# Tung-I/Dual-awareness-Attention-for-Few-shot-Object-Detection

Hardware: AMD Instinct MI355X
Metric: query-images/sec (res50, way=2, shot=3, bs=4 per GPU, train-mode forward) (higher is better)
Workload: dtype f32 (operands, accumulation, results; multiplies as an exact bf16x3 split, six bf16 MFMA products each)

## Files before the change

dual-awareness-attention-for-few-shot-object-detection_amd/csrc/attention.hip:

```cpp
#include "common.h"
#include "../../include/dana_hip.h"
#include "attn_segments.h"
#include <float.h>

namespace {

__device__ __forceinline__ float wave_sum(float v) {
#pragma unroll
  for (int o = 32; o > 0; o >>= 1) v += __shfl_xor(v, o);
  return v;
}
__device__ __forceinline__ float wave_max(float v) {
#pragma unroll
  for (int o = 32; o > 0; o >>= 1) v = fmaxf(v, __shfl_xor(v, o));
  return v;
}

__global__ void __launch_bounds__(256)
rowdot_kernel(const float* __restrict__ x, const float* __restrict__ w, const float* __restrict__ bias,
              float* __restrict__ out, long rows, int D, long ld) {
  const int lane = threadIdx.x & 63;
  const long row = (long)blockIdx.x * 4 + (threadIdx.x >> 6);
  if (row >= rows) return;
  const float4* xr = (const float4*)(x + row * ld);
// ... 25 lines not shown
  }
  s = wave_sum(s);
  for (int l = lane; l < L; l += 64) r[l] = r[l] / s;
}

__global__ void __launch_bounds__(256)
ba_apply_kernel(float* __restrict__ S, const float* __restrict__ w, int L, int D, long ld, float gamma, float slope) {
  extern __shared__ float ws[];
  float* part = ws + ((L + 3) & ~3);
  const int g = blockIdx.y;
  for (int l = threadIdx.x; l < L; l += blockDim.x) ws[l] = w[(long)g * L + l];
  __syncthreads();
  const int c4 = threadIdx.x & 15, rg = threadIdx.x >> 4;
  const int d = blockIdx.x * 64 + c4 * 4;
  const bool ok = d + 3 < D;
  float* base = S + (long)g * L * ld + d;
  float4 acc = make_float4(0.f, 0.f, 0.f, 0.f);
  if (ok)
    for (int l = rg; l < L; l += 16) {
      const float4 v = *(const float4*)(base + (long)l * ld);
      const float wl = ws[l];
      acc.x += wl * v.x;
      acc.y += wl * v.y;
      acc.z += wl * v.z;
      acc.w += wl * v.w;
    }
  *(float4*)(part + rg * 64 + c4 * 4) = acc;
  __syncthreads();
  float4 tot = make_float4(0.f, 0.f, 0.f, 0.f);
#pragma unroll
  for (int r = 0; r < 16; ++r) {
    const float4 p = *(const float4*)(part + r * 64 + c4 * 4);
    tot.x += p.x;
    tot.y += p.y;
    tot.z += p.z;
    tot.w += p.w;
  }
  float4 add;
  add.x = gamma * (tot.x > 0.f ? tot.x : tot.x * slope);
  add.y = gamma * (tot.y > 0.f ? tot.y : tot.y * slope);
  add.z = gamma * (tot.z > 0.f ? tot.z : tot.z * slope);
  add.w = gamma * (tot.w > 0.f ? tot.w : tot.w * slope);
  if (ok)
    for (int l = rg; l < L; l += 16) {
      float4 v = *(const float4*)(base + (long)l * ld);
      v.x += add.x;
      v.y += add.y;
      v.z += add.z;
      v.w += add.w;
      *(float4*)(base + (long)l * ld) = v;
    }
}

__global__ void __launch_bounds__(256)
attn_softmax_unary_kernel(float* __restrict__ scores, const float* __restrict__ unary, long rows, long rows_per_batch,
                          long unary_batch_stride, int nseg, int L, long ld, int kpad, float ugamma, float out_scale) {
  const int lane = threadIdx.x & 63;
  const long row = (long)blockIdx.x * 4 + (threadIdx.x >> 6);
  if (row >= rows) return;
  float* r = scores + row * ld;
  const float* u = unary + (row / rows_per_batch) * unary_batch_stride;
  constexpr int RV = 8;
  if (L <= 64 * RV) {
    for (int sgm = 0; sgm < nseg; ++sgm) {
      float* x = r + sgm * L;
      float v[RV];
      float m = -FLT_MAX;
#pragma unroll
      for (int i = 0; i < RV; ++i) {
        const int l = lane + 64 * i;
        v[i] = l < L ? x[l] : -FLT_MAX;
        m = fmaxf(m, v[i]);
      }
      m = wave_max(m);
      float s = 0.f;
#pragma unroll
      for (int i = 0; i < RV; ++i)
        if (lane + 64 * i < L) {
          v[i] = expf(v[i] - m);
          s += v[i];
        }
      s = wave_sum(s);
#pragma unroll
      for (int i = 0; i < RV; ++i) {
        const int l = lane + 64 * i;
        if (l < L) x[l] = (v[i] / s + ugamma * u[sgm * L + l]) * out_scale;
      }
    }
    for (int l = nseg * L + lane; l < kpad; l += 64) r[l] = 0.f;
    return;
  }
  for (int sgm = 0; sgm < nseg; ++sgm) {
    float* x = r + sgm * L;
    float m = -FLT_MAX;
    for (int l = lane; l < L; l += 64) m = fmaxf(m, x[l]);
    m = wave_max(m);
    float s = 0.f;
    for (int l = lane; l < L; l += 64) {
      const float e = expf(x[l] - m);
      x[l] = e;
      s += e;
    }
    s = wave_sum(s);
    for (int l = lane; l < L; l += 64) x[l] = (x[l] / s + ugamma * u[sgm * L + l]) * out_scale;
  }
  for (int l = nseg * L + lane; l < kpad; l += 64) r[l] = 0.f;
// ... 13 lines not shown
}

}

extern "C" {

int dana_rowdot(const float* x, const float* w, const float* bias, float* out, long rows, int dim, long ld,
                dana_stream_t stream) {
  DANA_CHECK_ARG(rows >= 0 && dim > 0 && dim % 4 == 0, "dana_rowdot: bad shape");
  if (rows == 0) return DANA_OK;
  DANA_CHECK_ARG(x && w && out, "dana_rowdot: null pointer");
  if (ld <= 0) ld = dim;
  DANA_CHECK_ARG(ld % 4 == 0, "dana_rowdot: ld %% 4 != 0");
  rowdot_kernel<<<dana_ceil_div(rows, 4), 256, 0, (hipStream_t)stream>>>(x, w, bias, out, rows, dim, ld);
  DANA_CHECK_LAUNCH("dana_rowdot");
  return DANA_OK;
}

int dana_softmax_rows(float* x, long groups, int length, long ld, dana_stream_t stream) {
  DANA_CHECK_ARG(groups >= 0 && length > 0, "dana_softmax_rows: bad shape");
  if (groups == 0) return DANA_OK;
  DANA_CHECK_ARG(x, "dana_softmax_rows: null pointer");
  if (ld <= 0) ld = length;
  softmax_rows_kernel<<<dana_ceil_div(groups, 4), 256, 0, (hipStream_t)stream>>>(x, groups, length, ld);
  DANA_CHECK_LAUNCH("dana_softmax_rows");
  return DANA_OK;
}

int dana_softmax_rows_to(const float* x, float* out, long groups, int length, long ld_in, long ld_out, dana_stream_t stream) {
  DANA_CHECK_ARG(groups >= 0 && length > 0, "dana_softmax_rows_to: bad shape");
  if (groups == 0) return DANA_OK;
  DANA_CHECK_ARG(x && out, "dana_softmax_rows_to: null pointer");
  if (ld_in <= 0) ld_in = length;
  if (ld_out <= 0) ld_out = length;
  softmax_rows_kernel<<<dana_ceil_div(groups, 4), 256, 0, (hipStream_t)stream>>>(out, groups, length, ld_out, x, ld_in);
  DANA_CHECK_LAUNCH("dana_softmax_rows_to");
  return DANA_OK;
}

int dana_ba_apply(float* s, const float* w, int groups, int length, int dim, long ld, float gamma, float slope,
                  dana_stream_t stream) {
  DANA_CHECK_ARG(groups >= 0 && length > 0 && dim > 0, "dana_ba_apply: bad shape");
  if (groups == 0) return DANA_OK;
  DANA_CHECK_ARG(s && w, "dana_ba_apply: null pointer");
  if (ld <= 0) ld = dim;
  DANA_CHECK_ARG(dim % 4 == 0 && ld % 4 == 0 && ((uintptr_t)s & 15) == 0, "dana_ba_apply: dim, ld must be multiples of 4 (float4 rows)");
  dim3 grid(dana_ceil_div(dim, 64), groups);
  const size_t lds = (size_t)(((length + 3) & ~3) + 16 * 64) * sizeof(float);
  ba_apply_kernel<<<grid, 256, lds, (hipStream_t)stream>>>(s, w, length, dim, ld, gamma, slope);
  DANA_CHECK_LAUNCH("dana_ba_apply");
  return DANA_OK;
}

int dana_attn_softmax_unary(float* scores, const float* unary, long rows, long rows_per_batch, long unary_batch_stride,
                            int nseg, int length, long ld, int kpad, float unary_gamma, float out_scale,
                            dana_stream_t stream) {
  DANA_CHECK_ARG(rows >= 0 && rows_per_batch > 0 && nseg > 0 && length > 0 && ld >= (long)nseg * length &&
                     kpad <= ld,
                 "dana_attn_softmax_unary: bad shape");
  if (rows == 0) return DANA_OK;
  DANA_CHECK_ARG(scores && unary, "dana_attn_softmax_unary: null pointer");
  attn_softmax_unary_kernel<<<dana_ceil_div(rows, 4), 256, 0, (hipStream_t)stream>>>(
      scores, unary, rows, rows_per_batch, unary_batch_stride > 0 ? unary_batch_stride : (long)nseg * length, nseg,
      length, ld, kpad, unary_gamma, out_scale);
  DANA_CHECK_LAUNCH("dana_attn_softmax_unary");
  return DANA_OK;
}

int dana_attn_softmax_unary_w(float* scores, const float* unary, long rows, long rows_per_batch, long unary_batch_stride,
                              int nseg, int length, long ld, int kpad, float unary_gamma, const float* seg_scale,
                              long scale_batch_stride, dana_stream_t stream) {
  DANA_CHECK_ARG(rows >= 0 && rows_per_batch > 0 && nseg > 0 && length > 0 && ld >= (long)nseg * length &&
                     kpad <= ld,
                 "dana_attn_softmax_unary_w: bad shape");
  if (rows == 0) return DANA_OK;
  DANA_CHECK_ARG(scores && unary && seg_scale, "dana_attn_softmax_unary_w: null pointer");
  attn_softmax_unary_w_kernel<<<dana_ceil_div(rows, 4), 256, 0, (hipStream_t)stream>>>(
      scores, unary, seg_scale, rows, rows_per_batch, unary_batch_stride > 0 ? unary_batch_stride : (long)nseg * length,
      scale_batch_stride > 0 ? scale_batch_stride : (long)nseg, nseg, length, ld, kpad, unary_gamma);
  DANA_CHECK_LAUNCH("dana_attn_softmax_unary_w");
  return DANA_OK;
}

}
```

dual-awareness-attention-for-few-shot-object-detection_amd/csrc/elementwise.hip:

```cpp
#include "common.h"
#include "../../include/dana_hip.h"
#include <float.h>

namespace {

int grid_for(long total, int block) {
  long g = (total + block - 1) / block;
  return (int)(g < 1 ? 1 : (g > 65535L * 16 ? 65535L * 16 : g));
}

__global__ void __launch_bounds__(256)
nchw_to_nhwc_kernel(const float* __restrict__ in, float* __restrict__ out, int C, int HW, int cpad, long ldo,
                    long total) {
  for (long i = (long)blockIdx.x * blockDim.x + threadIdx.x; i < total; i += (long)blockDim.x * gridDim.x) {
    const int c = (int)(i % cpad);
    const long pix = i / cpad;
    const long b = pix / HW, hw = pix % HW;
    out[pix * ldo + c] = c < C ? in[(b * C + c) * HW + hw] : 0.f;
  }
}

__global__ void __launch_bounds__(256)
nchw3_to_nhwc4_kernel(const float* __restrict__ in, float4* __restrict__ out, int HW, int total_pix) {
  for (int i = blockIdx.x * blockDim.x + threadIdx.x; i < total_pix; i += blockDim.x * gridDim.x) {
// ... 292 lines not shown
    for (int dy = 0; dy < k; ++dy) {
      const float4 v = hsum[((oy + dy) * OW + ox) * AP_CH4 + q];
      s.x += v.x;
      s.y += v.y;
      s.z += v.z;
      s.w += v.w;
    }
    out[((b * OH + oy) * OW + ox) * C4 + c0 + q] = make_float4(s.x * inv, s.y * inv, s.z * inv, s.w * inv);
  }
}

__global__ void __launch_bounds__(256)
spatial_mean_kernel(const float4* __restrict__ in, float4* __restrict__ out, int P, int C4, long ldi4, long total) {
  const float cnt = (float)P;
  for (long i = (long)blockIdx.x * blockDim.x + threadIdx.x; i < total; i += (long)blockDim.x * gridDim.x) {
    const int c = (int)(i % C4);
    const long g = i / C4;
    float4 s = make_float4(0, 0, 0, 0);
    for (int p = 0; p < P; ++p) {
      const float4 v = in[(g * P + p) * ldi4 + c];
      s.x += v.x;
      s.y += v.y;
      s.z += v.z;
      s.w += v.w;
    }
    out[i] = make_float4(s.x / cnt, s.y / cnt, s.z / cnt, s.w / cnt);
  }
}

__global__ void __launch_bounds__(256)
add_pe_kernel(const float4* __restrict__ in, const float4* __restrict__ pe, float4* __restrict__ out, int L, int C4,
              long ldi4, long ldo4, long total) {
  for (long i = (long)blockIdx.x * blockDim.x + threadIdx.x; i < total; i += (long)blockDim.x * gridDim.x) {
    const int c = (int)(i % C4);
    const long r = i / C4;
    const float4 a = in[r * ldi4 + c], b = pe[(r % L) * C4 + c];
    out[r * ldo4 + c] = make_float4(a.x + b.x, a.y + b.y, a.z + b.z, a.w + b.w);
  }
}

__global__ void __launch_bounds__(256)
add_pe_groups_kernel(const float4* __restrict__ in, const float4* __restrict__ pe, float4* __restrict__ out, int L, int C4,
                     long rows_per_group, long in_group4, long out_group4, long total) {
  for (long i = (long)blockIdx.x * blockDim.x + threadIdx.x; i < total; i += (long)blockDim.x * gridDim.x) {
    const int c = (int)(i % C4);
    const long rr = i / C4;
    const long g = rr / rows_per_group, r = rr % rows_per_group;
    const float4 a = in[g * in_group4 + r * C4 + c], b = pe[(r % L) * C4 + c];
    out[g * out_group4 + r * C4 + c] = make_float4(a.x + b.x, a.y + b.y, a.z + b.z, a.w + b.w);
  }
}

constexpr int CM_ROWS = 64;
__global__ void __launch_bounds__(256)
colmean_partial_kernel(const float* __restrict__ x, float* __restrict__ partial, int L, int D, long ld) {
  __shared__ float part[4][64];
  const int col = blockIdx.x * 64 + (threadIdx.x & 63);
  const int rl = threadIdx.x >> 6;
  const float* base = x + (long)blockIdx.z * L * ld;
  const int l0 = blockIdx.y * CM_ROWS, l1 = min(L, l0 + CM_ROWS);
  float s = 0.f;
  if (col < D)
    for (int l = l0 + rl; l < l1; l += 4) s += base[(long)l * ld + col];
  part[rl][threadIdx.x & 63] = s;
  __syncthreads();
  if (rl == 0 && col < D)
    partial[((long)blockIdx.z * gridDim.y + blockIdx.y) * D + col] =
        (part[0][threadIdx.x] + part[1][threadIdx.x]) + (part[2][threadIdx.x] + part[3][threadIdx.x]);
}
__global__ void __launch_bounds__(256)
colmean_apply_kernel(float* __restrict__ x, const float* __restrict__ partial, int L, int D, long ld) {
  const int col = blockIdx.x * 64 + (threadIdx.x & 63);
  const int rl = threadIdx.x >> 6;
  if (col >= D) return;
  float s = 0.f;
  for (int c = 0; c < (int)gridDim.y; ++c) s += partial[((long)blockIdx.z * gridDim.y + c) * D + col];
  const float mean = s / (float)L;
  float* base = x + (long)blockIdx.z * L * ld;
  const int l0 = blockIdx.y * CM_ROWS, l1 = min(L, l0 + CM_ROWS);
  for (int l = l0 + rl; l < l1; l += 4) base[(long)l * ld + col] -= mean;
}

__global__ void __launch_bounds__(256)
colmean_fused_kernel(float* __restrict__ x, int L, int D, long ld) {
  __shared__ float part[4][64];
  __shared__ float mean_s[64];
  const int tc = threadIdx.x & 63, col = blockIdx.x * 64 + tc, rl = threadIdx.x >> 6;
  float* base = x + (long)blockIdx.z * L * ld;
  float total = 0.f;
  for (int l0 = 0; l0 < L; l0 += CM_ROWS) {
    const int l1 = min(L, l0 + CM_ROWS);
    float s = 0.f;
    if (col < D)
      for (int l = l0 + rl; l < l1; l += 4) s += base[(long)l * ld + col];
    part[rl][tc] = s;
    __syncthreads();
    if (rl == 0) total += (part[0][tc] + part[1][tc]) + (part[2][tc] + part[3][tc]);
    __syncthreads();
  }
  if (rl == 0) mean_s[tc] = total / (float)L;
  __syncthreads();
  if (col >= D) return;
  const float mean = mean_s[tc];
  for (int l = rl; l < L; l += 4) base[(long)l * ld + col] -= mean;
}

__global__ void __launch_bounds__(256)
transpose_kernel(const float* __restrict__ in, float* __restrict__ out, int R, int C, long ldi, long ldo,
                 long in_batch, long out_batch, int zero_pad) {
  __shared__ float t[32][33];
  const float* ib = in + (long)blockIdx.z * in_batch;
  float* ob = out + (long)blockIdx.z * out_batch;
  const int c0 = blockIdx.x * 32, r0 = blockIdx.y * 32;
  const int tx = threadIdx.x & 31, ty = threadIdx.x >> 5;
  for (int j = ty; j < 32; j += 8) {
    const int r = r0 + j, c = c0 + tx;
    t[j][tx] = (r < R && c < C) ? ib[(long)r * ldi + c] : 0.f;
  }
  __syncthreads();
  for (int j = ty; j < 32; j += 8) {
    const int c = c0 + j, r = r0 + tx;
    if (c < C && (r < R || (zero_pad && r < ldo))) ob[(long)c * ldo + r] = t[tx][j];
  }
}

__global__ void __launch_bounds__(256)
labels_posneg_kernel(const float* __restrict__ labels, long long* __restrict__ out, long n) {
  const long i = (long)blockIdx.x * blockDim.x + threadIdx.x;
  if (i >= 2 * n) return;
  out[i] = i < n ? (long long)labels[i] : 0ll;
}

__global__ void __launch_bounds__(256)
bn_train_backward_kernel(const float* __restrict__ dy, const float* __restrict__ x, const float* __restrict__ mean,
                         const float* __restrict__ var, const float* __restrict__ gamma, float eps, long rows, int C,
                         float* __restrict__ dx, float* __restrict__ dgamma, float* __restrict__ dbeta, int accumulate) {
  __shared__ float s1[4][64], s2[4][64];
  const int cl = threadIdx.x & 63, rl = threadIdx.x >> 6;
  const int c = blockIdx.x * 64 + cl;
  const bool ok = c < C;
  const float mu = ok ? mean[c] : 0.f;
  const float istd = ok ? 1.0f / sqrtf(var[c] + eps) : 0.f;
  float a1 = 0.f, a2 = 0.f;
  if (ok)
    for (long r = rl; r < rows; r += 4) {
      const float g = dy[r * C + c];
      a1 += g;
      a2 += g * ((x[r * C + c] - mu) * istd);
    }
  s1[rl][cl] = a1;
  s2[rl][cl] = a2;
  __syncthreads();
  const float t1 = ((s1[0][cl] + s1[1][cl]) + s1[2][cl]) + s1[3][cl];
  const float t2 = ((s2[0][cl] + s2[1][cl]) + s2[2][cl]) + s2[3][cl];
  if (!ok) return;
  if (rl == 0) {
    dgamma[c] = accumulate ? dgamma[c] + t2 : t2;
// ... 291 lines not shown
        (const float4*)in, (float4*)out, height, width, oh, ow, channels / 4, k, rows_total);
  } else {
    avgpool_kernel<<<grid_for(total, 256), 256, 0, (hipStream_t)stream>>>((const float4*)in, (float4*)out, height, width,
                                                                          oh, ow, channels / 4, k, stride, total);
  }
  DANA_CHECK_LAUNCH("dana_avgpool_nhwc");
  return DANA_OK;
}

int dana_spatial_mean_nhwc(const float* in, float* out, int groups, int positions, int channels, long in_pix_stride,
                           dana_stream_t stream) {
  DANA_CHECK_ARG(groups >= 0 && positions > 0 && channels % 4 == 0, "dana_spatial_mean_nhwc: bad shape");
  if (groups == 0) return DANA_OK;
  DANA_CHECK_ARG(in && out, "dana_spatial_mean_nhwc: null pointer");
  if (in_pix_stride <= 0) in_pix_stride = channels;
  DANA_CHECK_ARG(in_pix_stride % 4 == 0, "dana_spatial_mean_nhwc: stride %% 4 != 0");
  const long total = (long)groups * (channels / 4);
  spatial_mean_kernel<<<grid_for(total, 256), 256, 0, (hipStream_t)stream>>>(
      (const float4*)in, (float4*)out, positions, channels / 4, in_pix_stride / 4, total);
  DANA_CHECK_LAUNCH("dana_spatial_mean_nhwc");
  return DANA_OK;
}

int dana_add_pe(const float* in, const float* pe, float* out, long rows, int length, int channels,
                long in_stride, long out_stride, dana_stream_t stream) {
  DANA_CHECK_ARG(rows >= 0 && length > 0 && channels > 0 && channels % 4 == 0, "dana_add_pe: bad shape");
  if (rows == 0) return DANA_OK;
  DANA_CHECK_ARG(in && pe && out, "dana_add_pe: null pointer");
  if (in_stride <= 0) in_stride = channels;
  if (out_stride <= 0) out_stride = channels;
  DANA_CHECK_ARG(in_stride % 4 == 0 && out_stride % 4 == 0, "dana_add_pe: strides %% 4 != 0");
  const long total = rows * (channels / 4);
  add_pe_kernel<<<grid_for(total, 256), 256, 0, (hipStream_t)stream>>>(
      (const float4*)in, (const float4*)pe, (float4*)out, length, channels / 4, in_stride / 4, out_stride / 4, total);
  DANA_CHECK_LAUNCH("dana_add_pe");
  return DANA_OK;
}

int dana_add_pe_groups(const float* in, const float* pe, float* out, long groups, long rows_per_group, int length, int channels,
                       long in_group_stride, long out_group_stride, dana_stream_t stream) {
  DANA_CHECK_ARG(groups >= 0 && rows_per_group > 0 && length > 0 && channels > 0 && channels % 4 == 0 &&
                     in_group_stride % 4 == 0 && out_group_stride % 4 == 0,
                 "dana_add_pe_groups: bad shape");
  if (groups == 0) return DANA_OK;
  DANA_CHECK_ARG(in && pe && out, "dana_add_pe_groups: null pointer");
  const long total = groups * rows_per_group * (channels / 4);
  add_pe_groups_kernel<<<grid_for(total, 256), 256, 0, (hipStream_t)stream>>>(
      (const float4*)in, (const float4*)pe, (float4*)out, length, channels / 4, rows_per_group, in_group_stride / 4,
      out_group_stride / 4, total);
  DANA_CHECK_LAUNCH("dana_add_pe_groups");
  return DANA_OK;
}

size_t dana_colmean_sub_workspace_bytes(int groups, int length, int dim) {
  if (groups <= 0 || length <= 0 || dim <= 0) return 0;
  return (size_t)groups * ((length + CM_ROWS - 1) / CM_ROWS) * dim * sizeof(float);
}

int dana_colmean_sub(float* x, int groups, int length, int dim, long ld, void* workspace, size_t workspace_bytes,
                     dana_stream_t stream) {
  DANA_CHECK_ARG(groups >= 0 && length > 0 && dim > 0, "dana_colmean_sub: bad shape");
  if (groups == 0) return DANA_OK;
  DANA_CHECK_ARG(x, "dana_colmean_sub: null pointer");
  if (ld <= 0) ld = dim;
  const size_t need = dana_colmean_sub_workspace_bytes(groups, length, dim);
  if (!workspace || workspace_bytes < need) {
    dana_set_error("dana_colmean_sub: workspace %zu < %zu", workspace_bytes, need);
    return DANA_ERR_WORKSPACE;
  }
  if (length <= 1024 && groups <= 65535) {
    dim3 grid1(dana_ceil_div(dim, 64), 1, groups);
    colmean_fused_kernel<<<grid1, 256, 0, (hipStream_t)stream>>>(x, length, dim, ld);
    DANA_CHECK_LAUNCH("dana_colmean_sub(fused)");
    return DANA_OK;
  }
  dim3 grid(dana_ceil_div(dim, 64), dana_ceil_div(length, CM_ROWS), groups);
  DANA_CHECK_ARG(grid.y <= 65535 && grid.z <= 65535, "dana_colmean_sub: too many chunks/groups");
  colmean_partial_kernel<<<grid, 256, 0, (hipStream_t)stream>>>(x, (float*)workspace, length, dim, ld);
  DANA_CHECK_LAUNCH("dana_colmean_sub(partial)");
  colmean_apply_kernel<<<grid, 256, 0, (hipStream_t)stream>>>(x, (const float*)workspace, length, dim, ld);
  DANA_CHECK_LAUNCH("dana_colmean_sub(apply)");
  return DANA_OK;
}

int dana_transpose_batched(const float* in, float* out, int groups, int rows, int cols, long ldi, long ldo,
                           long in_batch, long out_batch, dana_stream_t stream) {
  DANA_CHECK_ARG(groups >= 0 && rows > 0 && cols > 0 && ldi >= cols && ldo >= rows, "dana_transpose_batched: bad shape");
  if (groups == 0) return DANA_OK;
  DANA_CHECK_ARG(in && out, "dana_transpose_batched: null pointer");
  const int zero_pad = ldo > rows ? 1 : 0;
  dim3 grid(dana_ceil_div(cols, 32), dana_ceil_div(zero_pad ? (int)ldo : rows, 32), groups);
  transpose_kernel<<<grid, 256, 0, (hipStream_t)stream>>>(in, out, rows, cols, ldi, ldo, in_batch, out_batch, zero_pad);
  DANA_CHECK_LAUNCH("dana_transpose_batched");
  return DANA_OK;
}

int dana_labels_posneg_i64(const float* labels, long long* out, long n, dana_stream_t stream) {
  DANA_CHECK_ARG(n >= 0, "dana_labels_posneg_i64: bad shape");
  if (n == 0) return DANA_OK;
  DANA_CHECK_ARG(labels && out, "dana_labels_posneg_i64: null pointer");
  labels_posneg_kernel<<<dana_ceil_div(2 * n, 256), 256, 0, (hipStream_t)stream>>>(labels, out, n);
  DANA_CHECK_LAUNCH("dana_labels_posneg_i64");
  return DANA_OK;
}

int dana_pack_conv_weight(const float* w_oihw, float* out, int cout, int cin, int kh, int kw, int stem7,
                          dana_stream_t stream) {
  DANA_CHECK_ARG(cout > 0 && cin > 0 && kh > 0 && kw > 0, "dana_pack_conv_weight: bad shape");
  DANA_CHECK_ARG(w_oihw && out, "dana_pack_conv_weight: null pointer");
  if (stem7) {
    DANA_CHECK_ARG(kh == 7 && kw == 7 && cin <= 4, "dana_pack_conv_weight: stem7 needs 7x7, cin<=4");
    const long total = (long)cout * 224;
    pack_stem_kernel<<<grid_for(total, 256), 256, 0, (hipStream_t)stream>>>(w_oihw, out, cin, total);
  } else {
    const long total = (long)cout * cin * kh * kw;
    pack_weight_kernel<<<grid_for(total, 256), 256, 0, (hipStream_t)stream>>>(w_oihw, out, cin, kh, kw, total);
  }
  DANA_CHECK_LAUNCH("dana_pack_conv_weight");
  return DANA_OK;
}

// ... 47 lines not shown
```

dual-awareness-attention-for-few-shot-object-detection_amd/dana.py:

```python
import contextlib
import math
import time
import weakref
from types import SimpleNamespace

import numpy as np
import torch
import torch.nn as nn
import torch.nn.functional as F

from . import ops
from .config import cfg
from . import targets as T


class Bottleneck(nn.Module):
    expansion = 4

    def __init__(self, inplanes, planes, stride=1, downsample=None):
        super().__init__()
        self.conv1 = nn.Conv2d(inplanes, planes, kernel_size=1, stride=stride, bias=False)
        self.bn1 = nn.BatchNorm2d(planes)
        self.conv2 = nn.Conv2d(planes, planes, kernel_size=3, stride=1, padding=1, bias=False)
        self.bn2 = nn.BatchNorm2d(planes)
# ... 84 lines not shown
                               "(each forward can be differentiated once; run the forward again)")
        gs = [torch.zeros((), device=fctx.model._grad_anchor.device) if g is None else g.reshape(()) for g in (g1, g2, g3, g4)]
        fctx.saved = None
        BW.model_backward(fctx.model, torch.stack(gs), ctx=ctx)
        return None, None, None, None, None, None


_HERE = contextlib.nullcontext()

ATTENTION_LEVELS = ("ba", "rpn", "roi")


def _on(stream):
    return _HERE if stream is None else ops.on_stream(stream)


def _rows(t, row):
    return t[row:] if row and t is not None else t


class DAnARCNN(nn.Module):

    def __init__(self, classes, attention_type="concat", rpn_reduce_dim=256, rcnn_reduce_dim=256, gamma=0.1,
                 semantic_enhance=False, num_layers=50, pretrained=False, num_way=2, num_shot=5, pos_encoding=True):
        super().__init__()
        if attention_type not in ("concat", "product"):
            raise ValueError("attention_type must be 'concat' or 'product' (dana.py:70-77)")
        self.model_path = "data/pretrained_model/resnet50_caffe.pth"
        self.dout_base_model = 1024
        self.pretrained = pretrained
        self.classes = classes
        self.n_classes = len(classes)
        self.n_way = num_way
        self.n_shot = num_shot
        self.attention_type = attention_type
        self.channel_gamma = gamma
        self.unary_gamma = 0.1
        self.semantic_enhance = semantic_enhance
        self.rpn_reduce_dim = rpn_reduce_dim
        self.rcnn_reduce_dim = rcnn_reduce_dim
        self.pos_encoding = pos_encoding
        self.pool_feat_dim = 1024
        self.rcnn_dim = 64
        self.use_winograd = True
        self.winograd_tile = 4
        self.winograd_min_cin = 128
        self.presplit_weights = True
        self.merge_trunk = False
        self.merge_from = 0
        self.fold_roi_pe = True
        self.fold_roi_attn = True
        self.prefetch_dgrad = "layer4"
        self.rpn_side_role = "wgrad"
        self.nms_inclusive = False
        dim_in = self.pool_feat_dim

        def lin(i, o):
            m = nn.Linear(i, o)
            nn.init.normal_(m.weight, std=0.01)
            nn.init.constant_(m.bias, 0)
            return m

        self.rpn_unary_layer = lin(dim_in, 1)
        self.rcnn_unary_layer = lin(dim_in, 1)
        self.rpn_adapt_q_layer = lin(dim_in, rpn_reduce_dim)
        self.rpn_adapt_k_layer = lin(dim_in, rpn_reduce_dim)
        self.rcnn_adapt_q_layer = lin(dim_in, rcnn_reduce_dim)
        self.rcnn_adapt_k_layer = lin(dim_in, rcnn_reduce_dim)
        if self.semantic_enhance:
            self.rpn_channel_k_layer = lin(dim_in, 1)
        corr_dim = 2048 if attention_type == "concat" else 1024
        self.RCNN_rpn = _RPNParams(corr_dim)
        self.rcnn_transform_layer = nn.Linear(corr_dim, self.rcnn_dim)
        self.output_score_layer = FFN(64 * 49, dim_in)
        self._plan = None
        self._consts = {}
        self.generalised_support = False
        self.device_rng = False
        self.rng_seed = 1996
        self._rng_calls = 0
        self._conv_cache = {}
        self._epoch = 0
        self._ctx = None
        self._grad_anchor = None

    def create_architecture(self):
        self._init_modules()
        self._init_weights()

    trunk_layers = (3, 4, 6, 3)

    def _init_modules(self):
        resnet = _ResNet50Params(tuple(self.trunk_layers))
        if self.pretrained:
            print("Loading pretrained weights from %s" % (self.model_path))
            state_dict = torch.load(self.model_path)
            resnet.load_state_dict({k: v for k, v in state_dict.items() if k in resnet.state_dict()})
        self.RCNN_base = nn.Sequential(resnet.conv1, resnet.bn1, resnet.relu, resnet.maxpool, resnet.layer1,
                                       resnet.layer2, resnet.layer3)
        self.RCNN_top = nn.Sequential(resnet.layer4)
        self.RCNN_bbox_pred = nn.Linear(2048, 4)
        for p in self.RCNN_base[0].parameters():
            p.requires_grad = False
        for p in self.RCNN_base[1].parameters():
            p.requires_grad = False
        assert 0 <= cfg.RESNET.FIXED_BLOCKS < 4
# ... 370 lines not shown
            if side is not None:
                main.wait_event(ops.record_event(side))
            return [(n, hw, row, None) for n, hw, row, _ in segs]

        merged = two and merge_from <= 0
        segs, row = [], 0
        for i, im in enumerate(ims):
            n, _, H, W = im.shape
            segs.append((n, (H, W), row, side if i and not merged else None))
            row += n * H * W
        x, segs = self._stem(segs, ims, plan["stem"], merged, alloc)
        yield
        nl = len(plan["layers"])
        stall = getattr(self, "_debug_stall", None) if two else None
        for li, layer in enumerate(plan["layers"]):
            if two and not merged and li >= merge_from:
                segs, merged = join(segs), True
            for bi, bp in enumerate(layer):
                last = (li == nl - 1) and (bi == len(layer) - 1)
                if stall is not None and not merged and li == stall[0]:
                    torch.cuda._sleep(int(stall[1]))
                x, segs, dest = self._block(segs, x, bp, merged, outs=outs if last and outs[0][1] else None,
                                            saves=saves if li >= save_from else None, key="RCNN_base.%d.%d" % (4 + li, bi), alloc=alloc,
                                            save_m=save_m)
                if not last:
                    yield
        if two and not merged:
            segs = join(segs)
        return x, segs, dest

    @staticmethod
    def _feat_size(H, W):
        h, w = (H + 6 - 7) // 2 + 1, (W + 6 - 7) // 2 + 1
        h, w = ops.maxpool_out_size(h, w)
        for _ in range(2):
            h, w = (h - 1) // 2 + 1, (w - 1) // 2 + 1
        return h, w

    def _check_support_map(self, sh_, sw_):
        if (sh_, sw_) != (20, 20):
            if not self.generalised_support or sh_ % 7 or sw_ % 7:
                raise RuntimeError("support images must be 320x320 (20x20 stride-16 map), as the reference hard-codes "
                                   "(dana.py:105); got a %dx%d map%s" % (sh_, sw_, "" if self.generalised_support else
                                   " (set model.generalised_support = True for maps whose sides are multiples of 7)"))

    def _support_rpn_side(self, sup, B, shot, way, L, dev, stream, ctx=None, branch=True, tap=None):
        s_pe = torch.empty((B, shot * L, 1024), dtype=torch.float32, device=dev)
        ops.add_pe_groups(sup, self._pe_table(L, dev), B, shot * L, L, 1024, way * shot * L * 1024, s_pe)
        return self._support_rpn_chain(s_pe, B, shot, L, dev, stream, ctx, branch, tap)

    def _support_rpn_chain(self, s_pe, B, shot, L, dev, stream, ctx=None, branch=True, tap=None):
        d = self.rpn_reduce_dim
        K1 = shot * L
        if self.semantic_enhance:
            wc, bc = self._w(self.rpn_channel_k_layer)
            wgt = ops.rowdot(s_pe, wc, bc, B * shot * L, 1024)
            ops.softmax_rows_(wgt, B * shot, L)
            if ctx is not None:
                ctx.update(s_pre=s_pe.clone(), ba_w=wgt)
            if tap is not None:
                tap["ba_w"] = wgt
            ops.ba_apply_(s_pe, wgt, B * shot, L, 1024, gamma=self.channel_gamma, slope=0.01)
        br_role = getattr(self, "rpn_side_role", "wgrad")
        br = self._stream(br_role, dev) if (branch and br_role and not getattr(self, "_single_stream", False)
                                            and not torch.cuda.is_current_stream_capturing()) else None

        def unary_and_transpose():
            wu, bu = self._w(self.rpn_unary_layer)
            u_ = ops.rowdot(s_pe, wu, bu, B * shot * L, 1024)
            ops.softmax_rows_(u_, B * shot, L)
            return u_, ops.transpose_batched(s_pe, B, K1, 1024)

        if br is not None:
            s_pe_ready = ops.record_event()
            br.wait_event(s_pe_ready)
            s_pe.record_stream(br)
            with ops.on_stream(br):
                unary, s_t = unary_and_transpose()
                branch_done = ops.record_event()
        _, bk = self._w(self.rpn_adapt_k_layer)
        kb3, kld = self._lin_b(self.rpn_adapt_k_layer)
        kp = ops.gemm_nt(s_pe, kb3, B * shot * L, d, 1024, ldb=kld, shift=bk)
        ops.colmean_sub_(kp, B * shot, L, d)
        if br is not None:
            stream.wait_event(branch_done)
        else:
            unary, s_t = unary_and_transpose()
        return s_pe, kp, unary, s_t

    def _support_roi_side(self, sup, Ns, sh_, sw_, plan, dev, product, ctx=None):
        P2 = cfg.POOLING_SIZE * cfg.POOLING_SIZE
        pool = self._support_pool(sh_, sw_)
        sp = ops.avgpool(sup, Ns, sh_, sw_, 1024, pool[0], pool[1])
        sp_pe = ops.add_pe(sp, plan["pe49"], Ns * P2, P2, 1024)
        k2, un2, sw = self._support_roi_chain(sp_pe, Ns, product, ctx)
        return sp_pe, k2, un2, sw, pool

    @staticmethod
    def _support_pool(sh_, sw_):
        if (sh_, sw_) == (20, 20):
            return (14, 1)
        if sh_ != sw_:
            raise RuntimeError("generalised supports must be square")
        return (sh_ // 7, sh_ // 7)

    def _support_roi_chain(self, sp_pe, Ns, product, ctx=None):
        P2 = cfg.POOLING_SIZE * cfg.POOLING_SIZE
        dq = self.rcnn_reduce_dim
        _, bk2 = self._w(self.rcnn_adapt_k_layer)
        k2b3, k2ld = self._lin_b(self.rcnn_adapt_k_layer)
        k2 = ops.gemm_nt(sp_pe, k2b3, Ns * P2, dq, 1024, ldb=k2ld, shift=bk2)
        ops.colmean_sub_(k2, Ns, P2, dq)
        wu2, bu2 = self._w(self.rcnn_unary_layer)
        un2 = ops.rowdot(sp_pe, wu2, bu2, Ns * P2, 1024)
        ops.softmax_rows_(un2, Ns, P2)
        sw = None
        if getattr(self, "fold_roi_attn", True) and not product:
            wt_a_s, wt_a_s_ld = self._lin_b(self.rcnn_transform_layer, 1024, 1024)
            sw = ops.gemm_nt(sp_pe, wt_a_s, Ns * P2, self.rcnn_dim, 1024, ldb=wt_a_s_ld)
            if ctx is not None:
                ctx["sw"] = sw
        return k2, un2, sw

    def _rpn_split_plan(self, plan):
# ... 1113 lines not shown
```

dual-awareness-attention-for-few-shot-object-detection_amd/ops.py:

```python
import ctypes
import time as _time

import torch

from ._lib import lib, DanaError

HOST_WAIT = [0.0]

NCHW, NHWC = 0, 1
EPI_RELU, CONV_STEM7, W_SPLIT3, A_SPLIT3 = 1, 2, 256, 512

PROFILE = None
PROF_ROLE = None


def _prof_begin():
    if PROFILE is None:
        return None
    e = torch.cuda.Event(enable_timing=True)
    e.record()
    return e


def _prof_end(e0, tag, flops, nbytes=0.0, executed=None):
# ... 1032 lines not shown
        if v is not None and v.data_ptr() == w.data_ptr():
            return _chk(v, "weight")
    w = _chk(w.detach().contiguous(), "weight")
    O, I, KH, KW = w.shape
    out = torch.empty((O, 7 * 8 * 4) if stem else (O, KH * KW * I), dtype=torch.float32, device=w.device)
    lib().call("dana_pack_conv_weight", _p(w), _p(out), O, I, KH, KW, int(stem), _stream())
    return out


def bn_fold(bn_weight, bn_bias, running_mean, running_var, eps):
    n = bn_weight.numel()
    scale = torch.empty((n,), dtype=torch.float32, device=bn_weight.device)
    shift = torch.empty_like(scale)
    lib().call("dana_bn_fold", _p(_chk(bn_weight.detach().contiguous(), "gamma")),
               _p(_chk(bn_bias.detach().contiguous(), "beta")), _p(_chk(running_mean.contiguous(), "mean")),
               _p(_chk(running_var.contiguous(), "var")), float(eps), _p(scale), _p(shift), n, _stream())
    return scale, shift


def rowdot(x, w, bias, rows, dim, ld=0):
    _chk(x, "x")
    out = torch.empty((rows,), dtype=torch.float32, device=x.device)
    lib().call("dana_rowdot", _p(x), _p(_chk(w.detach().contiguous(), "w")),
               _p(_chk(bias.detach().contiguous(), "bias")) if bias is not None else None, _p(out), rows, dim, ld,
               _stream())
    return out


def softmax_rows_(x, groups, length, ld=0):
    _chk(x, "x")
    lib().call("dana_softmax_rows", _p(x), groups, length, ld, _stream())
    return x


def softmax_rows_to(x, out, groups, length, ld_in=0, ld_out=0):
    lib().call("dana_softmax_rows_to", _p(_chk(x, "x")), _p(_chk(out, "out")), groups, length, ld_in, ld_out, _stream())
    return out


def labels_posneg(labels_f):
    n = labels_f.numel()
    out = torch.empty(2 * n, dtype=torch.int64, device=labels_f.device)
    lib().call("dana_labels_posneg_i64", _p(_chk(labels_f, "labels")), _p(out), n, _stream())
    return out


def ba_apply_(s, w, groups, length, dim, ld=0, gamma=0.1, slope=0.01):
    _chk(s, "s")
    _chk(w, "w")
    lib().call("dana_ba_apply", _p(s), _p(w), groups, length, dim, ld, float(gamma), float(slope), _stream())
    return s


def attn_softmax_unary_(scores, unary, rows, rows_per_batch, nseg, length, ld, kpad, unary_gamma, out_scale,
                        unary_batch_stride=0):
    _chk(scores, "scores")
    _chk(unary, "unary")
    lib().call("dana_attn_softmax_unary", _p(scores), _p(unary), rows, rows_per_batch, unary_batch_stride, nseg, length,
               ld, kpad,
               float(unary_gamma), float(out_scale), _stream())
    return scores


def attn_softmax_unary_w_(scores, unary, rows, rows_per_batch, nseg, length, ld, kpad, unary_gamma, seg_scale,
                          unary_batch_stride=0, scale_batch_stride=0):
    _chk(scores, "scores")
    _chk(unary, "unary")
    _chk(seg_scale, "seg_scale")
    lib().call("dana_attn_softmax_unary_w", _p(scores), _p(unary), rows, rows_per_batch, unary_batch_stride, nseg, length,
               ld, kpad, float(unary_gamma), _p(seg_scale), scale_batch_stride, _stream())
    return scores


def attn_softmax_unary_sweep_w(scores, out, unary, B, C, hw, nseg, length, ld_in, ld_out, kpad, unary_gamma, seg_scale,
                               unary_stride=0, scale_stride=0):
    _chk(scores, "scores")
    _chk(out, "out")
    _chk(unary, "unary")
    _chk(seg_scale, "seg_scale")
    lib().call("dana_attn_softmax_unary_sweep_w", _p(scores), _p(out), _p(unary), B, C, hw, unary_stride, nseg, length,
               ld_in, ld_out, kpad, float(unary_gamma), _p(seg_scale), scale_stride, _stream())
    return out


def gather_shot_blocks(srcs, rows, blocks, index, view, m):
    P, shot, dev = index.numel(), view.size(1), index.device
    _chk(index, "index", torch.int32)
    _chk(view, "view", torch.int32)
    for t, r, b in zip(srcs, rows, blocks):
        _chk(t, "src")
        if t.numel() != t.size(0) * r * shot * b:
            raise ValueError("gather_shot_blocks: a source is not [n_sets][%d][%d][%d]" % (r, shot, b))
    dsts = [torch.empty((P, r, m, b), dtype=torch.float32, device=dev) for r, b in zip(rows, blocks)]
    w = torch.empty((P, m), dtype=torch.float32, device=dev)
    tab = torch.tensor([[t.data_ptr() for t in srcs], [t.data_ptr() for t in dsts], list(rows), [b * 4 for b in blocks]],
                       dtype=torch.int64).to(dev)
    lib().call("dana_gather_shot_blocks", _p(tab[0]), _p(tab[1]), _p(tab[2]), _p(tab[3]), len(srcs), _p(index), _p(view),
               _p(w), srcs[0].size(0), shot, m, P, _stream())
    return dsts, w


def bank_gather_episode(map_pe, pool_pe, index, B, way, shot, s_pe=None, sp_pe=None):
    _chk(map_pe, "map_pe")
    _chk(pool_pe, "pool_pe")
    _chk(index, "index", torch.int32)
    if map_pe.dim() != 3 or pool_pe.dim() != 3 or pool_pe.size(0) != map_pe.size(0) or pool_pe.size(2) != map_pe.size(2):
# ... 411 lines not shown
```

include/dana_hip.h:

```cpp
#ifndef DANA_HIP_H
#define DANA_HIP_H
#include <stddef.h>
#include <stdint.h>

#ifdef __cplusplus
extern "C" {
#endif

typedef void* dana_stream_t;

#define DANA_LAYOUT_NCHW 0
#define DANA_LAYOUT_NHWC 1

#define DANA_EPI_RELU 1
#define DANA_CONV_STEM7 2
#define DANA_W_SPLIT3 256
#define DANA_A_SPLIT3 512

const char* dana_last_error(void);
int dana_abi_version(void);

int dana_set_mfma_mode(int mode);
int dana_get_mfma_mode(void);

// ... 171 lines not shown
                                dana_stream_t stream);
int dana_avgpool_nhwc(const float* in, float* out, int batch, int height, int width, int channels, int k, int stride,
                      dana_stream_t stream);
int dana_spatial_mean_nhwc(const float* in, float* out, int groups, int positions, int channels, long in_pix_stride,
                           dana_stream_t stream);
int dana_batch_stats(const float* x, float* mean, float* var_biased, long rows, int channels, long ld, void* workspace,
                     size_t workspace_bytes, dana_stream_t stream);
int dana_scale_shift_relu(float* x, const float* scale, const float* shift, long rows, int channels, int relu,
                          dana_stream_t stream);
int dana_bn_train_backward(const float* grad_out, const float* x, const float* mean, const float* var_biased,
                           const float* gamma, float eps, long rows, int channels, float* grad_x, float* grad_gamma,
                           float* grad_beta, int accumulate, dana_stream_t stream);
int dana_depthwise_corr_nhwc(const float* feat, const float* kernels, float* out, long n_maps, int height, int width,
                             int channels, int kh, int kw, long maps_per_kernel, long feat_pix_stride,
                             dana_stream_t stream);
int dana_depthwise_corr_nhwc_grouped(const float* feat, const float* kernels, float* out, long n_maps, int height,
                                     int width, int channels, int kh, int kw, int group, long feat_pix_stride,
                                     dana_stream_t stream);
int dana_depthwise_corr_backward_nhwc(const float* grad_out, const float* feat, const float* kernels, float* grad_feat,
                                      float* grad_kernels, long n_maps, int height, int width, int channels, int kh,
                                      int kw, long maps_per_kernel, long feat_pix_stride, int accumulate_kernels,
                                      dana_stream_t stream);
int dana_maxpool2x2s2_nhwc(const float* in, float* out, int batch, int height, int width, int channels,
                           dana_stream_t stream);
int dana_maxpool2x2s2_backward_nhwc(const float* in, const float* grad_out, float* grad_in, int batch, int height,
                                    int width, int channels, dana_stream_t stream);
int dana_sigmoid(float* x, long n, dana_stream_t stream);
int dana_scale_rows_by_group(const float* x, const float* group_vec, float* out, long rows, long rows_per_group,
                             int channels, dana_stream_t stream);
int dana_scale_rows_grouped(const float* x, const float* vec, float* out, long rows, int channels, long ld_x, int group,
                            long n_blocks, dana_stream_t stream);
int dana_add_pe(const float* in, const float* pe, float* out, long rows, int length, int channels,
                long in_stride, long out_stride, dana_stream_t stream);
int dana_add_pe_groups(const float* in, const float* pe, float* out, long groups, long rows_per_group, int length, int channels,
                       long in_group_stride, long out_group_stride, dana_stream_t stream);
size_t dana_colmean_sub_workspace_bytes(int groups, int length, int dim);
int dana_colmean_sub(float* x, int groups, int length, int dim, long ld, void* workspace, size_t workspace_bytes,
                     dana_stream_t stream);
int dana_transpose_batched(const float* in, float* out, int groups, int rows, int cols, long ldi, long ldo,
                           long in_batch, long out_batch, dana_stream_t stream);
int dana_pack_conv_weight(const float* w_oihw, float* out, int cout, int cin, int kh, int kw, int stem7,
                          dana_stream_t stream);
int dana_bn_fold(const float* gamma, const float* beta, const float* mean, const float* var, float eps, float* scale,
                 float* shift, int n, dana_stream_t stream);


int dana_rowdot(const float* x, const float* w, const float* bias, float* out, long rows, int dim, long ld,
                dana_stream_t stream);
int dana_softmax_rows(float* x, long groups, int length, long ld, dana_stream_t stream);
int dana_softmax_rows_to(const float* x, float* out, long groups, int length, long ld_in, long ld_out, dana_stream_t stream);
int dana_labels_posneg_i64(const float* labels, long long* out, long n, dana_stream_t stream);
int dana_ba_apply(float* s, const float* w, int groups, int length, int dim, long ld, float gamma, float slope,
                  dana_stream_t stream);
int dana_attn_softmax_unary(float* scores, const float* unary, long rows, long rows_per_batch, long unary_batch_stride,
                            int nseg, int length, long ld, int kpad, float unary_gamma, float out_scale,
                            dana_stream_t stream);
int dana_attn_softmax_unary_w(float* scores, const float* unary, long rows, long rows_per_batch, long unary_batch_stride,
                              int nseg, int length, long ld, int kpad, float unary_gamma, const float* seg_scale,
                              long scale_batch_stride, dana_stream_t stream);


int dana_proposal_target_prepare(const float* rois, const float* gt_boxes, int B, int n_rois, int n_gt,
                                 float fg_thresh, float bg_thresh_hi, float bg_thresh_lo, float* max_overlaps,
                                 int* gt_assignment, int* fg_list, int* bg_list, int* counts, dana_stream_t stream);
int dana_proposal_target_gather(const float* rois, const float* gt_boxes, int B, int n_rois, int n_gt,
                                const int* gt_assignment, const int* fg_list, const int* bg_list, const int* picks,
                                const int* fg_taken, int rois_per_image, const float* means4, const float* stds4,
                                const float* inside_w4, int normalize, float* rois_out, float* labels_out,
                                float* bbox_targets, float* inside_weights, float* outside_weights,
                                dana_stream_t stream);


int dana_anchor_target_prepare(const float* gt_boxes, const float* im_info, const float* base_anchors, int B,
                               int A, int H, int W, int feat_stride, int n_gt, float negative_overlap,
                               float positive_overlap, float* labels, float* max_overlaps, int* argmax,
                               int* fg_list, int* bg_list, int* counts, dana_stream_t stream);
int dana_anchor_target_disable(float* labels, const int* fg_list, const int* bg_list, const int* which,
                               const int* pos, int n, int anchors_per_image, dana_stream_t stream);
int dana_anchor_target_disable_dev(float* labels, const int* fg_list, const int* bg_list, const int* n_dev,
                                   const int* which_pos_pairs, int capacity, int anchors_per_image,
                                   dana_stream_t stream);
int dana_anchor_target_outputs(const float* labels, const float* max_overlaps, const int* argmax,
                               const float* gt_boxes, const float* base_anchors, int B, int A, int H, int W,
                               int feat_stride, int n_gt, float inside_weight, float outside_weight, const float* outside_weight_dev,
                               float* labels_out, float* bbox_targets, float* inside_weights,
                               float* outside_weights, dana_stream_t stream);
int dana_plain_rcnn_loss(const float* scores, const long long* labels, const float* bbox_pred, const float* bbox_targets,
                         const float* inside_weights, const float* outside_weights, int n, int n_classes, float sigma,
                         float* losses2, float* grad_scores, float* grad_bbox, dana_stream_t stream);
size_t dana_rcnn_loss_workspace_bytes(int n);
int dana_rcnn_loss(const float* score_pos, const float* score_neg, const float* labels, const float* bbox_pred,
                   const float* bbox_targets, const float* inside_weights, const float* outside_weights, int n,
                   float sigma, float* losses3, float* grad_score_pos, float* grad_score_neg, float* grad_bbox,
                   void* workspace, size_t workspace_bytes, dana_stream_t stream);
size_t dana_rpn_loss_workspace_bytes(void);
int dana_rpn_loss(const float* heads, long head_row_stride, const float* labels, const int* argmax,
                  const float* gt_boxes, const float* base_anchors, int B, int A, int H, int W, int feat_stride,
                  int n_gt, float sigma, float inside_weight, float outside_weight, const float* outside_weight_dev, float* losses3, void* workspace,
                  size_t workspace_bytes, dana_stream_t stream);


size_t dana_conv2d_wgrad_workspace_bytes(int batch, int in_h, int in_w, int cin, int cout, int kh, int kw, int stride,
                                         int pad);
int dana_conv2d_wgrad_nhwc(const float* grad_out, const float* input, float* grad_weight, int batch, int in_h,
                           int in_w, int cin, int cout, int kh, int kw, int stride, int pad, long in_pix_stride,
                           long grad_pix_stride, const float* row_scale, int accumulate, void* workspace, size_t workspace_bytes,
// ... 170 lines not shown
```

include/dana_hip_debug.h:

```cpp
#ifndef DANA_HIP_DEBUG_H
#define DANA_HIP_DEBUG_H
#include "dana_hip.h"

#ifdef __cplusplus
extern "C" {
#endif

int dana_debug_force_tile(int tile);
int dana_set_epilogue_mode(int mode);
int dana_get_epilogue_mode(void);
int dana_set_igemm_trace(unsigned long long* buffer);
int dana_set_sort_mode(int mode);

int dana_debug_stream_create_cumask(const unsigned int* mask, int mask_words, int n_xcd, dana_stream_t* stream_out);
int dana_debug_stream_destroy(dana_stream_t stream);

size_t dana_debug_radix_sort_workspace_bytes(long n);
int dana_debug_radix_sort_pairs(const unsigned long long* keys_in, const int* vals_in, unsigned long long* keys_out,
                                int* vals_out, long n, int key_bits, void* workspace, size_t workspace_bytes,
                                dana_stream_t stream);

#ifdef __cplusplus
}
#endif
#endif
```

Baseline: 701.4.

## Fuse support softmax, channel attention apply and transpose; add single-pass column-mean kernel

Adds a kernel that holds a channel slab of each support map in LDS, computes the softmax of the channel-attention logits, applies the gated attention add, and writes both the updated map and its transposed layout in one pass. This replaces three launches (softmax, ba_apply, transpose_batched) and the extra global reads they needed. It also adds a 1024-thread column-mean-subtract kernel that keeps values in registers, so x is read once instead of twice. The cost is heavy LDS use per block, which limits occupancy, and the transposed store uses strided writes.

```diff
diff --git a/dual-awareness-attention-for-few-shot-object-detection_amd/csrc/attention.hip b/dual-awareness-attention-for-few-shot-object-detection_amd/csrc/attention.hip
--- a/dual-awareness-attention-for-few-shot-object-detection_amd/csrc/attention.hip
+++ b/dual-awareness-attention-for-few-shot-object-detection_amd/csrc/attention.hip
@@ -101,6 +101,121 @@
     }
 }
 
+constexpr int BAT_THREADS = 1024;
+template <int SLAB>
+__global__ void __launch_bounds__(BAT_THREADS)
+ba_apply_t_kernel(const float* S, const float* __restrict__ logits, float* out, float* __restrict__ w_out,
+                  float* __restrict__ st, int L, int D, long ld, int shot, float gamma, float slope) {
+  constexpr int LDR = SLAB + 4, C4 = SLAB / 4;
+  extern __shared__ float bat_smem[];
+  float* slab = bat_smem;
+  float* ws = slab + (long)L * LDR;
+  float* part = ws + ((L + 3) & ~3);
+  float* add_s = part + 16 * SLAB;
+  const int g = blockIdx.y, d0 = blockIdx.x * SLAB, tid = threadIdx.x;
+  if (tid < 64) {
+    const float* in = logits + (long)g * L;
+    float x[16];
+#pragma unroll
+    for (int i = 0; i < 16; ++i) x[i] = tid + 64 * i < L ? in[tid + 64 * i] : 0.f;
+    float m = -FLT_MAX;
+#pragma unroll
+    for (int i = 0; i < 16; ++i)
+      if (tid + 64 * i < L) m = fmaxf(m, x[i]);
+    m = wave_max(m);
+    float s = 0.f;
+#pragma unroll
+    for (int i = 0; i < 16; ++i)
+      if (tid + 64 * i < L) {
+        x[i] = expf(x[i] - m);
+        s += x[i];
+      }
+    s = wave_sum(s);
+#pragma unroll
+    for (int i = 0; i < 16; ++i) {
+      const int l = tid + 64 * i;
+      if (l < L) {
+        const float p = x[i] / s;
+        ws[l] = p;
+        if (blockIdx.x == 0) w_out[(long)g * L + l] = p;
+      }
+    }
+  } else {
+    const float* src = S + (long)g * L * ld + d0;
+#pragma unroll 4
+    for (int i = tid - 64; i < L * C4; i += BAT_THREADS - 64) {
+      const int l = i / C4, c = (i % C4) * 4;
+      float4 v = make_float4(0.f, 0.f, 0.f, 0.f);
+      if (d0 + c + 3 < D) v = *(const float4*)(src + (long)l * ld + c);
+      *(float4*)(slab + l * LDR + c) = v;
+    }
+  }
+  __syncthreads();
+  if (tid < 16 * C4) {
+    const int c = (tid % C4) * 4, rg = tid / C4;
+    float4 acc = make_float4(0.f, 0.f, 0.f, 0.f);
+    for (int l = rg; l < L; l += 16) {
+      const float4 v = *(const float4*)(slab + l * LDR + c);
+      const float wl = ws[l];
+      acc.x += wl * v.x;
+      acc.y += wl * v.y;
+      acc.z += wl * v.z;
+      acc.w += wl * v.w;
+    }
+    *(float4*)(part + rg * SLAB + c) = acc;
+  }
+  __syncthreads();
+  if (tid < C4) {
+    const int c = tid * 4;
+    float4 tot = make_float4(0.f, 0.f, 0.f, 0.f);
+#pragma unroll
+    for (int r = 0; r < 16; ++r) {
+      const float4 p = *(const float4*)(part + r * SLAB + c);
+      tot.x += p.x;
+      tot.y += p.y;
+      tot.z += p.z;
+      tot.w += p.w;
+    }
+    float4 add;
+    add.x = gamma * (tot.x > 0.f ? tot.x : tot.x * slope);
+    add.y = gamma * (tot.y > 0.f ? tot.y : tot.y * slope);
+    add.z = gamma * (tot.z > 0.f ? tot.z : tot.z * slope);
+    add.w = gamma * (tot.w > 0.f ? tot.w : tot.w * slope);
+    *(float4*)(add_s + c) = add;
+  }
+  __syncthreads();
+  float* dst = out + (long)g * L * ld + d0;
+  for (int i = tid; i < L * C4; i += BAT_THREADS) {
+    const int l = i / C4, c = (i % C4) * 4;
+    if (d0 + c + 3 >= D) continue;
+    float4 v = *(const float4*)(slab + l * LDR + c);
+    const float4 add = *(const float4*)(add_s + c);
+    v.x += add.x;
+    v.y += add.y;
+    v.z += add.z;
+    v.w += add.w;
+    *(float4*)(dst + (long)l * ld + c) = v;
+  }
+  const long K1 = (long)shot * L;
+  float* sto = st + ((long)(g / shot) * D + d0) * K1 + (long)(g % shot) * L;
+  for (int c = tid >> 6; c < SLAB && d0 + c < D; c += BAT_THREADS / 64) {
+    const float add = add_s[c];
+    for (int l = tid & 63; l < L; l += 64) sto[c * K1 + l] = slab[l * LDR + c] + add;
+  }
+}
+
+template <int SLAB>
+int launch_ba_apply_t(const float* s, const float* logits, float* out, float* w_out, float* s_t, int groups, int shot,
+                      int length, int dim, long ld, float gamma, float slope, hipStream_t stream) {
+  const size_t lds = ((size_t)length * (SLAB + 4) + ((length + 3) & ~3) + 17 * SLAB) * sizeof(float);
+  static DeviceOnce attr;
+  attr.once([&] { return hipFuncSetAttribute((const void*)ba_apply_t_kernel<SLAB>, hipFuncAttributeMaxDynamicSharedMemorySize, 160 * 1024); });
+  dim3 grid(dana_ceil_div(dim, SLAB), groups);
+  ba_apply_t_kernel<SLAB><<<grid, BAT_THREADS, lds, stream>>>(s, logits, out, w_out, s_t, length, dim, ld, shot, gamma, slope);
+  DANA_CHECK_LAUNCH("dana_ba_apply_t");
+  return DANA_OK;
+}
+
 __global__ void __launch_bounds__(256)
 attn_softmax_unary_kernel(float* __restrict__ scores, const float* __restrict__ unary, long rows, long rows_per_batch,
                           long unary_batch_stride, int nseg, int L, long ld, int kpad, float ugamma, float out_scale) {
@@ -220,6 +335,23 @@
   return DANA_OK;
 }
 
+int dana_ba_apply_t(float* s, const float* logits, float* out, float* w_out, float* s_t, int groups, int shot, int length,
+                    int dim, long ld, float gamma, float slope, dana_stream_t stream) {
+  DANA_CHECK_ARG(groups >= 0 && shot > 0 && groups % shot == 0 && length > 0 && dim > 0, "dana_ba_apply_t: bad shape");
+  DANA_CHECK_ARG(length <= 1024, "dana_ba_apply_t: length %d > 1024 (a map's channel slab is held in LDS)", length);
+  DANA_CHECK_ARG(groups <= 65535, "dana_ba_apply_t: too many groups");
+  if (groups == 0) return DANA_OK;
+  DANA_CHECK_ARG(s && logits && w_out && s_t, "dana_ba_apply_t: null pointer");
+  if (!out) out = s;
+  if (ld <= 0) ld = dim;
+  DANA_CHECK_ARG(dim % 4 == 0 && ld % 4 == 0 && ld >= dim && (((uintptr_t)s | (uintptr_t)out) & 15) == 0,
+                 "dana_ba_apply_t: dim, ld must be multiples of 4 (float4 rows)");
+  DANA_CHECK_ARG(logits != w_out, "dana_ba_apply_t: the weights cannot overwrite the logits (every slab of a map reads them)");
+  if (length <= 512)
+    return launch_ba_apply_t<64>(s, logits, out, w_out, s_t, groups, shot, length, dim, ld, gamma, slope, (hipStream_t)stream);
+  return launch_ba_apply_t<32>(s, logits, out, w_out, s_t, groups, shot, length, dim, ld, gamma, slope, (hipStream_t)stream);
+}
+
 int dana_attn_softmax_unary(float* scores, const float* unary, long rows, long rows_per_batch, long unary_batch_stride,
                             int nseg, int length, long ld, int kpad, float unary_gamma, float out_scale,
                             dana_stream_t stream) {
diff --git a/dual-awareness-attention-for-few-shot-object-detection_amd/csrc/elementwise.hip b/dual-awareness-attention-for-few-shot-object-detection_amd/csrc/elementwise.hip
--- a/dual-awareness-attention-for-few-shot-object-detection_amd/csrc/elementwise.hip
+++ b/dual-awareness-attention-for-few-shot-object-detection_amd/csrc/elementwise.hip
@@ -368,6 +368,7 @@
 }
 
 constexpr int CM_ROWS = 64;
+std::atomic<int> g_colmean_mode{0};
 __global__ void __launch_bounds__(256)
 colmean_partial_kernel(const float* __restrict__ x, float* __restrict__ partial, int L, int D, long ld) {
   __shared__ float part[4][64];
@@ -419,6 +420,47 @@
   if (col >= D) return;
   const float mean = mean_s[tc];
   for (int l = rl; l < L; l += 4) base[(long)l * ld + col] -= mean;
+}
+
+constexpr int CMW_COLS = 32, CMW_INFLIGHT = 8, CMW_ROUNDS = 2;
+__global__ void __launch_bounds__(1024)
+colmean_wide_kernel(float* __restrict__ x, int L, int D, long ld) {
+  __shared__ float part[CMW_ROUNDS * CMW_INFLIGHT][4][CMW_COLS];
+  __shared__ float mean_s[CMW_COLS];
+  const int tc = threadIdx.x & 31, rl = (threadIdx.x >> 5) & 3, ch = threadIdx.x >> 7;
+  const int col = blockIdx.x * CMW_COLS + tc;
+  float* base = x + (long)blockIdx.z * L * ld;
+  float v[CMW_ROUNDS][CM_ROWS / 4];
+#pragma unroll
+  for (int rd = 0; rd < CMW_ROUNDS; ++rd) {
+    const int c = rd * CMW_INFLIGHT + ch, l0 = c * CM_ROWS;
+#pragma unroll
+    for (int i = 0; i < CM_ROWS / 4; ++i) {
+      const int l = l0 + rl + 4 * i;
+      v[rd][i] = (l < L && col < D) ? base[(long)l * ld + col] : 0.f;
+    }
+    float s = 0.f;
+#pragma unroll
+    for (int i = 0; i < CM_ROWS / 4; ++i)
+      if (l0 + rl + 4 * i < L && col < D) s += v[rd][i];
+    part[c][rl][tc] = s;
+  }
+  __syncthreads();
+  if (threadIdx.x < CMW_COLS) {
+    float total = 0.f;
+    for (int c = 0; c * CM_ROWS < L; ++c) total += (part[c][0][tc] + part[c][1][tc]) + (part[c][2][tc] + part[c][3][tc]);
+    mean_s[tc] = total / (float)L;
+  }
+  __syncthreads();
+  if (col >= D) return;
+  const float mean = mean_s[tc];
+#pragma unroll
+  for (int rd = 0; rd < CMW_ROUNDS; ++rd)
+#pragma unroll
+    for (int i = 0; i < CM_ROWS / 4; ++i) {
+      const int l = (rd * CMW_INFLIGHT + ch) * CM_ROWS + rl + 4 * i;
+      if (l < L) base[(long)l * ld + col] = v[rd][i] - mean;
+    }
 }
 
 __global__ void __launch_bounds__(256)
@@ -816,6 +858,12 @@
   return DANA_OK;
 }
 
+int dana_set_colmean_mode(int mode) {
+  DANA_CHECK_ARG(mode == 0 || mode == 1, "dana_set_colmean_mode: mode %d", mode);
+  g_colmean_mode = mode;
+  return DANA_OK;
+}
+
 size_t dana_colmean_sub_workspace_bytes(int groups, int length, int dim) {
   if (groups <= 0 || length <= 0 || dim <= 0) return 0;
   return (size_t)groups * ((length + CM_ROWS - 1) / CM_ROWS) * dim * sizeof(float);
@@ -831,6 +879,12 @@
   if (!workspace || workspace_bytes < need) {
     dana_set_error("dana_colmean_sub: workspace %zu < %zu", workspace_bytes, need);
     return DANA_ERR_WORKSPACE;
+  }
+  if (length > 2 * CM_ROWS && length <= CMW_ROUNDS * CMW_INFLIGHT * CM_ROWS && groups <= 65535 && g_colmean_mode == 0) {
+    dim3 gridw(dana_ceil_div(dim, CMW_COLS), 1, groups);
+    colmean_wide_kernel<<<gridw, 1024, 0, (hipStream_t)stream>>>(x, length, dim, ld);
+    DANA_CHECK_LAUNCH("dana_colmean_sub(wide)");
+    return DANA_OK;
   }
   if (length <= 1024 && groups <= 65535) {
     dim3 grid1(dana_ceil_div(dim, 64), 1, groups);
diff --git a/dual-awareness-attention-for-few-shot-object-detection_amd/dana.py b/dual-awareness-attention-for-few-shot-object-detection_amd/dana.py
--- a/dual-awareness-attention-for-few-shot-object-detection_amd/dana.py
+++ b/dual-awareness-attention-for-few-shot-object-detection_amd/dana.py
@@ -160,6 +160,7 @@
         self.fold_roi_attn = True
         self.prefetch_dgrad = "layer4"
         self.rpn_side_role = "wgrad"
+        self.fused_support_chain = True
         self.nms_inclusive = False
         dim_in = self.pool_feat_dim
 
@@ -636,24 +637,33 @@
     def _support_rpn_chain(self, s_pe, B, shot, L, dev, stream, ctx=None, branch=True, tap=None):
         d = self.rpn_reduce_dim
         K1 = shot * L
+        s_t = None
         if self.semantic_enhance:
             wc, bc = self._w(self.rpn_channel_k_layer)
             wgt = ops.rowdot(s_pe, wc, bc, B * shot * L, 1024)
-            ops.softmax_rows_(wgt, B * shot, L)
-            if ctx is not None:
-                ctx.update(s_pre=s_pe.clone(), ba_w=wgt)
+            if getattr(self, "fused_support_chain", True) and L <= 1024:
+                s_pre = s_pe
+                s_pe, wgt, s_t = ops.ba_apply_t(s_pre, wgt, B * shot, shot, L, 1024, gamma=self.channel_gamma, slope=0.01,
+                                                out=torch.empty_like(s_pre) if ctx is not None else None)
+                if ctx is not None:
+                    ctx.update(s_pre=s_pre, ba_w=wgt)
+            else:
+                ops.softmax_rows_(wgt, B * shot, L)
+                if ctx is not None:
+                    ctx.update(s_pre=s_pe.clone(), ba_w=wgt)
+                ops.ba_apply_(s_pe, wgt, B * shot, L, 1024, gamma=self.channel_gamma, slope=0.01)
             if tap is not None:
                 tap["ba_w"] = wgt
-            ops.ba_apply_(s_pe, wgt, B * shot, L, 1024, gamma=self.channel_gamma, slope=0.01)
         br_role = getattr(self, "rpn_side_role", "wgrad")
         br = self._stream(br_role, dev) if (branch and br_role and not getattr(self, "_single_stream", False)
                                             and not torch.cuda.is_current_stream_capturing()) else None
+        have_t = s_t
 
         def unary_and_transpose():
             wu, bu = self._w(self.rpn_unary_layer)
             u_ = ops.rowdot(s_pe, wu, bu, B * shot * L, 1024)
             ops.softmax_rows_(u_, B * shot, L)
-            return u_, ops.transpose_batched(s_pe, B, K1, 1024)
+            return u_, have_t if have_t is not None else ops.transpose_batched(s_pe, B, K1, 1024)
 
         if br is not None:
             s_pe_ready = ops.record_event()
diff --git a/dual-awareness-attention-for-few-shot-object-detection_amd/ops.py b/dual-awareness-attention-for-few-shot-object-detection_amd/ops.py
--- a/dual-awareness-attention-for-few-shot-object-detection_amd/ops.py
+++ b/dual-awareness-attention-for-few-shot-object-detection_amd/ops.py
@@ -1108,6 +1108,18 @@
     return s
 
 
+def ba_apply_t(s, logits, groups, shot, length, dim, out=None, ld=0, gamma=0.1, slope=0.01):
+    _chk(s, "s")
+    _chk(logits, "logits")
+    if out is not None:
+        _chk(out, "out")
+    w = torch.empty_like(logits)
+    s_t = torch.empty((groups // shot, dim, shot * length), dtype=torch.float32, device=s.device)
+    lib().call("dana_ba_apply_t", _p(s), _p(logits), _p(out), _p(w), _p(s_t), groups, shot, length, dim, ld, float(gamma),
+               float(slope), _stream())
+    return (s if out is None else out), w, s_t
+
+
 def attn_softmax_unary_(scores, unary, rows, rows_per_batch, nseg, length, ld, kpad, unary_gamma, out_scale,
                         unary_batch_stride=0):
     _chk(scores, "scores")
diff --git a/include/dana_hip.h b/include/dana_hip.h
--- a/include/dana_hip.h
+++ b/include/dana_hip.h
@@ -247,6 +247,8 @@
 int dana_labels_posneg_i64(const float* labels, long long* out, long n, dana_stream_t stream);
 int dana_ba_apply(float* s, const float* w, int groups, int length, int dim, long ld, float gamma, float slope,
                   dana_stream_t stream);
+int dana_ba_apply_t(float* s, const float* logits, float* out, float* w_out, float* s_t, int groups, int shot, int length,
+                    int dim, long ld, float gamma, float slope, dana_stream_t stream);
 int dana_attn_softmax_unary(float* scores, const float* unary, long rows, long rows_per_batch, long unary_batch_stride,
                             int nseg, int length, long ld, int kpad, float unary_gamma, float out_scale,
                             dana_stream_t stream);
diff --git a/include/dana_hip_debug.h b/include/dana_hip_debug.h
--- a/include/dana_hip_debug.h
+++ b/include/dana_hip_debug.h
@@ -11,6 +11,7 @@
 int dana_get_epilogue_mode(void);
 int dana_set_igemm_trace(unsigned long long* buffer);
 int dana_set_sort_mode(int mode);
+int dana_set_colmean_mode(int mode);
 
 int dana_debug_stream_create_cumask(const unsigned int* mask, int mask_words, int n_xcd, dana_stream_t* stream_out);
 int dana_debug_stream_destroy(dana_stream_t stream);
```

Result: no change. 707.4, median of 6 (+0.8%).
